# uber-research/vargp

Hardware: AMD Instinct MI355X
Metric: ELBO steps/sec (higher is better)
Workload: dtype f32; 1 GPU; BASELINE config 2 (Split-MNIST t=0): S3 F10 C10 M100 D784 B512 ELBO step; S_per_gpu=3, Mt=100, S_total=3, F=10, C=10, M=100, D=784, B=512, N=12000, optimizer=yogi, parallelism=sample-parallel x1, steps_per_graph_launch=10, launch=hipGraph replay

## Files before the change

vargp_amd/csrc/chol_blk16.h:

```cpp
#pragma once
#include "common.h"
#include <type_traits>

namespace vargp {

#ifdef VARGP_CB16_STAMPS
__device__ unsigned long long g_cb16_stamps[4][8][4];
extern "C" void vargp_debug_cb16_stamps(unsigned long long* out) { (void)hipMemcpyFromSymbol(out, HIP_SYMBOL(g_cb16_stamps), sizeof(g_cb16_stamps)); }
#define CB_STAMP(step, i) do { if (lane == 0 && blockIdx.x == 0) g_cb16_stamps[WV][step][i] = __builtin_amdgcn_s_memtime(); } while (0)
#else
#define CB_STAMP(step, i) do { } while (0)
#endif
typedef float cb_f32x4 __attribute__((ext_vector_type(4)));
constexpr int kCbNB = 7;
constexpr int kCbRD = 0;
constexpr int kCbWB = kCbRD + kCbNB * 256;
constexpr int kCbDD = kCbWB + 16 * 20;
constexpr int kCbED = kCbDD + 256;
constexpr int kCbLdsFloats = kCbED + 16;

template <int I, int N, class F>
__device__ __forceinline__ void cb_for(F&& f) {
  if constexpr (I < N) { f(std::integral_constant<int, I>{}); cb_for<I + 1, N>(f); }
}
__host__ __device__ constexpr int cb_owner(int c) { return c >= 3 ? 6 - c : c + 1; }
template <int WV> struct CbOwn {
  static constexpr int UA = 6 - WV, UB = WV > 0 ? WV - 1 : -1;
  static constexpr int XA = WV, XB = WV > 0 ? 7 - WV : -1;
  __host__ __device__ static constexpr bool owns_u(int c) { return c == UA || c == UB; }
  __host__ __device__ static constexpr bool owns_x(int c) { return c == XA || c == XB; }
  __host__ __device__ static constexpr int ui(int c, int k) { return c == UA ? k : (UA + 1) + k; }
  __host__ __device__ static constexpr int xi(int c, int i) { return c == XA ? i - XA : (7 - XA) + (i - XB); }
};

__device__ __forceinline__ void cb_mfma4(cb_f32x4& acc, const float4 a, const cb_f32x4 b) {
  acc = __builtin_amdgcn_mfma_f32_16x16x4f32(a.x, b[0], acc, 0, 0, 0);
  acc = __builtin_amdgcn_mfma_f32_16x16x4f32(a.y, b[1], acc, 0, 0, 0);
  acc = __builtin_amdgcn_mfma_f32_16x16x4f32(a.z, b[2], acc, 0, 0, 0);
  acc = __builtin_amdgcn_mfma_f32_16x16x4f32(a.w, b[3], acc, 0, 0, 0);
}
__device__ __forceinline__ void cb_barrier() { asm volatile("s_waitcnt lgkmcnt(0)\n\ts_barrier" ::: "memory"); }
__device__ __forceinline__ float cb_lane(float v, int lane) {
  return __int_as_float(__builtin_amdgcn_readlane(__float_as_int(v), lane));
}

template <int WV>
__device__ __forceinline__ void cb16_wave(float* __restrict__ stage, const int LS, double* __restrict__ sq, double* __restrict__ sd,
                                          const int n, const float eps, const int lane, int* __restrict__ flag, float* __restrict__ dump, int& fail) {
  using O = CbOwn<WV>;
  const int c = lane & 15, q = lane >> 4;
  cb_f32x4 accU[kCbNB], accX[kCbNB];
  cb_for<0, kCbNB>([&](auto ii) {
    constexpr int i = decltype(ii)::value;
    if constexpr (O::owns_u(i)) {
// ... 183 lines not shown
```

vargp_amd/csrc/common.h:

```cpp
#pragma once
#include <hip/hip_runtime.h>
#include <stdint.h>
#include <stdio.h>
#include <functional>
#include "../../include/vargp_hip.h"

#if defined(__HIPCC__)
namespace vargp {
constexpr int kSpanEnds = 4096;
struct SpanGuard {
  unsigned long long* p;
  unsigned long long* e;
  __device__ __forceinline__ SpanGuard(unsigned long long* q, unsigned long long* ends, int on) : p(on ? q : nullptr), e(ends) {
    if (p && threadIdx.x == 0 && blockIdx.x == 0 && blockIdx.y == 0 && blockIdx.z == 0) {
      p[0] = wall_clock64();
      p[2] = __builtin_amdgcn_s_memtime();
    }
  }
  __device__ __forceinline__ ~SpanGuard() {
    if (p && threadIdx.x == 0) {
      const unsigned lin = (blockIdx.z * gridDim.y + blockIdx.y) * gridDim.x + blockIdx.x;
      if (lin == 0) p[3] = __builtin_amdgcn_s_memtime();
      e[lin & (kSpanEnds - 1)] = wall_clock64();
    }
// ... 260 lines not shown
                     int D, int64_t Dp, int S, float kappa, int accumulate, hipStream_t st);

int chol_inv_bwd_first(const float* T, const float* gT, int nbatch, int n, void* ws, size_t ws_bytes,
                       const GemmParams* other, int oA, int oB, int onb, hipStream_t st);
int chol_inv_bwd_impl(const float* L, const float* T, const float* gL, const float* gT, float* gA, int nbatch, int n,
                      void* ws, size_t ws_bytes, bool gl_lower, hipStream_t st, bool first_done);

struct BwdMatArgs {
  const float* QP;
  const float *TT, *LL, *gQP, *RK, *KS, *seeds;
  const float* gTT;
  float *gKS, *Wuu, *r_uu, *gtheta;
  float *g_u_mean, *gLu_part;
  float* gL_acc;
  int S, C, M, D, NR, LD;
};
int launch_bwdmat_gemm(const BwdMatArgs& a, int first, int nmat, const GemmParams& p, int nbatch, hipStream_t st,
                       const char* tag, int* queue);

bool prof_remembering();
void prof_remember(const char* tag, std::function<void(hipStream_t)> relaunch);

struct ProfScope {
  ProfScope(const char* tag, hipStream_t st);
  ~ProfScope();
  int slot_;
  hipStream_t st_;
};

}
// ... 1 lines not shown
```

vargp_amd/csrc/elbo_t0.hip:

```cpp
#include <atomic>
#include <mutex>
#include <unordered_map>

#include "common.h"
STEP_SPAN_TABLE(t0)
#include "elbo_shared.h"
#include "t0_bwd_mid.h"
#include "t0_bwd_mid_multi.h"
#include "chol_gram.h"
#include "t0_prologue.h"
#include "t0_bwd_tail.h"

namespace vargp {

constexpr int kKuuSplit = 2;
#ifndef VARGP_KL_ROWS
#define VARGP_KL_ROWS 8
#endif
constexpr int kT0TileUnitsMax = 16384;
constexpr int kTailLdsDefault = 1;
constexpr int kKlRows = VARGP_KL_ROWS;


struct T0Ws {
// ... 850 lines not shown
                "%s: native noise needs rng_counter, eps_theta == eps_f == NULL and a sample offset >= 0", who);
  VARGP_REQUIRE(d->map_est ? d->S == 1
                           : (d->log_logvar && d->prior_log_mean && d->prior_log_logvar && (native || d->eps_theta)),
                "%s: hyper-parameter arguments inconsistent with map_est", who);
  VARGP_REQUIRE(d->ws_bytes >= vargp_elbo_t0_workspace_bytes(d->S, d->C, d->M, d->D, d->B, d->F),
                "%s: workspace too small", who);
  return VARGP_OK;
}

struct T0Tune {
  static long long env(const char* name, long long dflt) { const char* e = getenv(name); return e ? atoll(e) : dflt; }
  int64_t units = env("VARGP_T0_UNITS", kT0TileUnitsMax);
  int unmerge = env("VARGP_T0_UNMERGE", -1), side = env("VARGP_T0_SIDE", 1);
  int multi = env("VARGP_T0_MULTI", 0), parts = env("VARGP_T0_PARTS", 0);
  int fused = env("VARGP_T0_FUSED", 1), fused_bwd = env("VARGP_T0_FUSED_BWD", 1), mat_bwd = env("VARGP_T0_MAT_BWD", 1);
  int fold_small = env("VARGP_T0_FOLD_SMALL", 1);
  int front = env("VARGP_T0_FRONT", 1), gram_in_chain = env("VARGP_T0_GRAM_IN_CHAIN", -1), su = env("VARGP_T0_SU", 1);
  int tail = env("VARGP_T0_TAIL", 1), tail_lds = env("VARGP_T0_TAIL_LDS", kTailLdsDefault);
  int kuf_tile = env("VARGP_T0_KUF_TILE", 0), puf_tile = env("VARGP_T0_PUF_TILE", 0), puu_tile = env("VARGP_T0_PUU_TILE", 0);
  int kuu_split = env("VARGP_KUU_SPLIT", kKuuSplit), chol_f32 = env("VARGP_CHOL_F32", kCholF32Default);
};
static const T0Tune& t0_tune() { static const T0Tune tune; return tune; }

constexpr float kFwdMidSetup = 0.5f;
constexpr float kBwdMidSetup = 0.35f;
static int t0_tile_parts(int64_t SC, int ntile, int cus, float setup, int forced) {
  if (forced > 0) return forced < ntile ? forced : ntile;
  if (SC * ntile <= cus) return ntile;
  int best = ntile;
  float best_t = 1e30f;
  for (int np = 1; np <= ntile; ++np) {
    const float t = (float)cdiv(SC * np, (int64_t)cus) * (setup + (float)cdiv(ntile, np));
    if (t < best_t - 1e-6f) { best_t = t; best = np; }
  }
  return best;
}

struct T0Plan {
  bool native, generic_lik, unscaled_lik_grad, defer_softmax, fwd_softmax16;
  bool direct_gram, merge_chol, split_kuu, front, gram_in_chain, su_in_chain, fused_mid, fwd_multi, w_vec4;
  bool unmerge, side;
  bool fused_bwd, mat_bwd, bwd_multi, fused_tail, tail_lds;
  int kuf_tile, puf_tile, puu_tile;
  bool fold_small;
  int fold_roles, fold_extra;
  int ksp, ntile, fwd_parts, bwd_parts;
};
static T0Plan t0_plan(const vargp_elbo_t0_desc* d, const T0Ws& o, int cus) {
  const T0Tune& tune = t0_tune();
  const int S = d->S, C = d->C, M = d->M, D = d->D, B = d->B, F = d->F, LD = o.LD;
  const int64_t SC = (int64_t)S * C;
  const bool zx_aligned = ((reinterpret_cast<uintptr_t>(d->z) | reinterpret_cast<uintptr_t>(d->x)) & 15) == 0;
  T0Plan p{};
  p.native = t0_native(d);
  p.unscaled_lik_grad = C <= 16 && !d->ext_lik;
  p.generic_lik = C > 16 && !d->ext_lik;
  p.ntile = cdiv(B, 64);
// ... 15 lines not shown
  const bool units_ok = SC * p.ntile <= tune.units;
  p.fused_mid = tune.fused && M <= kFusedK && (M % 4) == 0 && (LD % 4) == 0 && units_ok;
  p.fwd_parts = t0_tile_parts(SC, p.ntile, cus, kFwdMidSetup, tune.parts);
  p.fwd_multi = p.fwd_parts < p.ntile || tune.multi == 1;
  p.w_vec4 = B % 4 == 0;
  {
    const int nsur = (int)(8 * cdiv(SC, 8) - SC) * p.ntile, need = (int)cdiv(SC, 2);
    p.fold_extra = nsur >= need ? 0 : (int)round_up(need - nsur, 8);
    p.fold_roles = nsur + p.fold_extra;
    p.fold_small = tune.fold_small && p.fused_mid && !p.fwd_multi && p.w_vec4 && !p.unmerge && M >= 4 &&
                   SC * p.ntile + std::min<int64_t>(p.fold_roles, SC) <= cus;
    if (!p.fold_small) p.fold_roles = p.fold_extra = 0;
  }
  p.fused_bwd = tune.fused_bwd && M <= kBmKP && M >= 4 && (M % 4) == 0 && (LD % 4) == 0 && (B % 4) == 0 && units_ok;
  p.mat_bwd = p.fused_bwd && tune.mat_bwd && (D % 4) == 0 && S <= kTailSMax && zx_aligned;
  p.bwd_parts = t0_tile_parts(SC, p.ntile, cus, kBwdMidSetup, tune.parts);
  p.bwd_multi = p.fused_bwd && (p.bwd_parts < p.ntile || tune.multi == 1);
  p.defer_softmax = d->defer_softmax && p.unscaled_lik_grad && p.fused_bwd && !p.bwd_multi && F <= 4 * kBmSmF && C <= kBmSmC &&
                    reinterpret_cast<uintptr_t>(p.native ? o.eps_f : d->eps_f) % 16 == 0;
  p.fwd_softmax16 = p.unscaled_lik_grad && !p.defer_softmax;
  p.fused_tail = p.mat_bwd && tune.tail && S <= kTailSMax;
  p.tail_lds = p.fused_tail && ((S > 4 && tune.tail_lds) || tune.tail_lds == 2);
  return p;
}

enum { kT0NoClear = 0, kT0Cleared = 1, kT0Consumed = 2, kT0SoftmaxDeferred = 16  };
static std::mutex g_t0_state_mu;
static std::unordered_map<const void*, int> g_t0_state;
static void t0_state_set(const void* ws, int v) {
  std::lock_guard<std::mutex> lock(g_t0_state_mu);
// ... 279 lines not shown
    ElboGemm gp{flat_gemm(o.QP + 4, LD, MLD, o.gW, B, MB, o.gQP + NR, LD, MLD, M, B, M), 0, 0, SC, "t0_gp_gemm"};
    gp.p.triA = 1;
    rc = run_gemm_pair(gg, gp.onto_c(), "t0_gg_gp_gemm", st);
    if (rc) return rc;
    rc = gt_gemm(false).run(st);
    if (rc) return rc;
    const ElboGemm grk = grk_gemm(NR + B);
    rc = chol_inv_bwd_first(o.TT, o.gTT, SC + C, M, o.chol, o.chol_bytes, &grk.p, grk.tA, grk.tB, grk.nbatch, st);
    if (rc) return rc;
  }
  if (plan.mat_bwd) {
    BwdMatArgs ma{};
    ma.QP = o.QP; ma.TT = o.TT; ma.LL = o.LL; ma.gQP = o.gQP; ma.RK = o.RK; ma.KS = o.KS; ma.seeds = seeds; ma.gTT = o.gTT;
    ma.gKS = o.gKS; ma.Wuu = o.Wuu; ma.r_uu = o.r_uu; ma.gtheta = o.gtheta;
    ma.g_u_mean = g_u_mean; ma.gLu_part = o.gLL;
    ma.S = S; ma.C = C; ma.M = M; ma.D = D; ma.NR = NR; ma.LD = LD;
    GemmParams puf = puf_gemm();
    if (plan.unmerge) {
      SideFork fork(st, plan.side);
      ma.gL_acc = o.gLL + SC * MM;
      rc = launch_bwdmat_gemm(ma, 0, SC, puf, 0, fork.side(), "t0_bwdmat_kuu", nullptr);
      if (rc) return rc;
      rc = launch_bwdmat_gemm(ma, SC, C, puf, 0, fork.side(), "t0_bwdmat_su", nullptr);
      if (rc) return rc;
      puf.tile = plan.puf_tile;
      rc = launch_gemm(puf, 0, 0, S, false, st, "rbf_kuf_bwd_product");
      if (rc) return rc;
      rc = fork.join();
    } else {
      rc = launch_bwdmat_gemm(ma, 0, SC + C, puf, S, st, "rbf_kuf_bwd_gemm", reinterpret_cast<int*>(o.queue));
    }
// ... 108 lines not shown
```

vargp_amd/csrc/gemm.hip:

```cpp
#include "common.h"
#include "chol_small3.h"
#include "t0_bwd_mat.h"
#include "t0_prologue.h"
#include <atomic>
#include <stdlib.h>
#include <string.h>
#include <type_traits>

STEP_SPAN_TABLE(gemm)
#ifdef STEP_SPANS
__device__ unsigned long long g_bmat_ends[64][2];
extern "C" void vargp_debug_bmat_ends(unsigned long long* out) { (void)hipMemcpyFromSymbol(out, HIP_SYMBOL(g_bmat_ends), sizeof(g_bmat_ends)); }
#endif

namespace vargp {

typedef float f32x16 __attribute__((ext_vector_type(16)));

__device__ float g_gemm_trash[512];

template <bool KC, int ROWS, int BK>
struct LdsLayout {
  static constexpr int kStride = KC ? BK : (ROWS + 4);
  static constexpr int kSize = KC ? ROWS * BK : BK * (ROWS + 4);
// ... 1294 lines not shown
  return check_launch("gemm_pair2");
}

static bool gemm_persist_ok(const GemmParams& p, int BK, bool AKC, bool BKC) {
  const int64_t extA = AKC ? ((int64_t)(p.M - 1) * p.lda + p.K) : ((int64_t)(p.K - 1) * p.lda + p.M);
  const int64_t extB = BKC ? ((int64_t)(p.N - 1) * p.ldb + p.K) : ((int64_t)(p.K - 1) * p.ldb + p.N);
  return gemm_vec_ok(p) && p.K >= 4 * BK && p.K % BK == 0 && !p.D && p.triA == 0 && p.triB == 0 && p.triC == 0 && !p.symout &&
         p.splitk <= 1 && (AKC || (p.M % 4 == 0 && p.M >= 4)) && (BKC || (p.N % 4 == 0 && p.N >= 4)) &&
         extA < (1ll << 29) && extB < (1ll << 29);
}

int launch_bwdmat_gemm(const BwdMatArgs& a, int first, int nmat, const GemmParams& p, int nbatch, hipStream_t st,
                       const char* tag, int* queue) {
  VARGP_REQUIRE(gemm_vec_ok(p), "bwdmat_gemm: the product's operands must be 16-byte aligned with strides % 4 == 0");
  VARGP_REQUIRE(a.M <= kBmKP && a.M >= 4 && (a.M % 4) == 0 && (a.LD % 4) == 0, "bwdmat_gemm: M = %d out of range", a.M);
  static_assert(kBwdMatLdsBytes >= sizeof(float) * gemm_lds_floats<64, 64, 64, true, false>(), "LDS of the GEMM role");
  if (prof_remembering() && strcmp(tag, "replay") != 0) {
    const GemmParams pc = p;
    const BwdMatArgs ac = a;
    prof_remember(tag, [=](hipStream_t s) { launch_bwdmat_gemm(ac, first, nmat, pc, nbatch, s, "replay", nullptr); });
  }
  static std::atomic<unsigned> attr_mask[2] = {};
  int dev = 0;
  VARGP_REQUIRE(hipGetDevice(&dev) == hipSuccess && dev >= 0 && dev < 64, "bwdmat_gemm: hipGetDevice failed");
  if (!((attr_mask[dev >> 5].load(std::memory_order_acquire) >> (dev & 31)) & 1u)) {
    VARGP_REQUIRE(hipFuncSetAttribute(reinterpret_cast<const void*>(t0_bwdmat_gemm_kernel),
                                      hipFuncAttributeMaxDynamicSharedMemorySize, (int)kBwdMatLdsBytes) == hipSuccess,
                  "bwdmat_gemm: cannot reserve %zu bytes of LDS", kBwdMatLdsBytes);
    attr_mask[dev >> 5].fetch_or(1u << (dev & 31), std::memory_order_release);
  }
// ... 88 lines not shown
```

vargp_amd/csrc/t0_bwd_mat.h:

```cpp
#pragma once
#include "t0_bwd_common.h"

namespace vargp {

constexpr int kMatS = 108;
constexpr int kMatN = kBmKP * kMatS;
constexpr size_t kBwdMatLdsBytes = sizeof(float) * (3 * kMatN + 4 * 128 + 8);

enum { kFamL = 0, kFamR = 1, kFamC = 2, kFamF = 3 };
constexpr unsigned kNone = 0xFFu;
__host__ __device__ constexpr unsigned mat_blk(int rb, int cb) { return (unsigned)((rb << 2) | cb); }
__host__ __device__ constexpr unsigned mat_blk4(unsigned a, unsigned b, unsigned c, unsigned d) {
  return a | (b << 8) | (c << 16) | (d << 24);
}
__host__ __device__ constexpr unsigned mat_blocks(int family, int wave) {
  return family == kFamL
             ? (wave == 0   ? mat_blk4(mat_blk(3, 3), mat_blk(0, 0), mat_blk(1, 0), kNone)
                : wave == 1 ? mat_blk4(mat_blk(2, 2), mat_blk(1, 1), kNone, kNone)
                : wave == 2 ? mat_blk4(mat_blk(3, 2), mat_blk(2, 1), kNone, kNone)
                            : mat_blk4(mat_blk(3, 1), mat_blk(2, 0), mat_blk(3, 0), kNone))
         : family == kFamR
             ? (wave == 0   ? mat_blk4(mat_blk(0, 0), mat_blk(3, 0), mat_blk(3, 1), kNone)
                : wave == 1 ? mat_blk4(mat_blk(1, 0), mat_blk(2, 0), kNone, kNone)
                : wave == 2 ? mat_blk4(mat_blk(1, 1), mat_blk(2, 1), kNone, kNone)
                            : mat_blk4(mat_blk(2, 2), mat_blk(3, 2), mat_blk(3, 3), kNone))
         : family == kFamC
             ? (wave == 0   ? mat_blk4(mat_blk(0, 0), mat_blk(1, 1), kNone, kNone)
                : wave == 1 ? mat_blk4(mat_blk(1, 0), mat_blk(2, 1), kNone, kNone)
                : wave == 2 ? mat_blk4(mat_blk(2, 0), mat_blk(3, 1), kNone, kNone)
                            : mat_blk4(mat_blk(3, 0), mat_blk(2, 2), mat_blk(3, 2), mat_blk(3, 3)))
             : (wave == 0   ? mat_blk4(mat_blk(0, 0), mat_blk(0, 1), mat_blk(3, 0), mat_blk(3, 1))
                : wave == 1 ? mat_blk4(mat_blk(0, 2), mat_blk(0, 3), mat_blk(3, 2), mat_blk(3, 3))
                : wave == 2 ? mat_blk4(mat_blk(1, 0), mat_blk(1, 1), mat_blk(2, 0), mat_blk(2, 1))
                            : mat_blk4(mat_blk(1, 2), mat_blk(1, 3), mat_blk(2, 2), mat_blk(2, 3)));
}
template <int FAM, int WV, int U> struct MatBlk {
  static constexpr unsigned code = (mat_blocks(FAM, WV) >> (8 * U)) & 0xFFu;
  static constexpr bool valid = code != kNone;
  static constexpr int rb = valid ? (int)(code >> 2) : 0, cb = valid ? (int)(code & 3u) : 0;
  static constexpr int GE = kBmKP / 8;
  static constexpr int g0 = FAM == kFamL ? 0 : (FAM == kFamC ? 4 * cb : 4 * rb);
  static constexpr int g1 = FAM == kFamL ? bm_min(GE, 4 * cb + 4) : GE;
};

template <bool AKC, bool BKC, int RB, int CB, int G0, int G1>
__device__ __forceinline__ void mat_block(bm_f32x16& acc, const float* __restrict__ sA, const float* __restrict__ sB, int li, int lh) {
  const int ia = min(32 * RB + li, kBmKP - 1), ib = min(32 * CB + li, kBmKP - 1);
  const float* pa = AKC ? sA + ia * kMatS + 4 * lh : sA + (4 * lh) * kMatS + ia;
  const float* pb = BKC ? sB + ib * kMatS + 4 * lh : sB + (4 * lh) * kMatS + ib;
  auto fa = [&](int g) { return AKC ? bm_frag_kc(pa, 8 * g) : bm_frag_km(pa, 8 * g, kMatS); };
  auto fb = [&](int g) { return BKC ? bm_frag_kc(pb, 8 * g) : bm_frag_km(pb, 8 * g, kMatS); };
  float4 a = fa(G0), b = fb(G0);
  bm_for<G0, G1>([&](auto gi) {
    constexpr int g = decltype(gi)::value;
    const float4 ca = a, cbv = b;
    if constexpr (g + 1 < G1) { a = fa(g + 1); b = fb(g + 1); }
    bm_mfma4(acc, ca, cbv);
  });
}

template <bool AKC, bool BKC, int FAM, int WV>
__device__ __forceinline__ void mat_product(bm_f32x16 (&acc)[4], const float* __restrict__ sA, const float* __restrict__ sB,
                                            bool zero, int li, int lh) {
  bm_for<0, 4>([&](auto ui) {
    constexpr int u = decltype(ui)::value;
    using Bk = MatBlk<FAM, WV, u>;
    if constexpr (Bk::valid) {
      if (zero) {
#pragma unroll
        for (int r = 0; r < 16; ++r) acc[u][r] = 0.f;
      }
      mat_block<AKC, BKC, Bk::rb, Bk::cb, Bk::g0, Bk::g1>(acc[u], sA, sB, li, lh);
    }
  });
}
template <int FAM, int WV, class F>
__device__ __forceinline__ void mat_foreach(int li, int lh, F&& f) {
  bm_for<0, 4>([&](auto ui) {
    constexpr int u = decltype(ui)::value;
    using Bk = MatBlk<FAM, WV, u>;
    if constexpr (Bk::valid) {
#pragma unroll
      for (int r = 0; r < 16; ++r) f(u, Bk::rb, Bk::cb, r, 32 * Bk::rb + (r & 3) + 8 * (r >> 2) + 4 * lh, 32 * Bk::cb + li);
    }
  });
}

__device__ __forceinline__ void mat_store(float* __restrict__ dst, const float4 (&src)[kBmNA], int M, int tid) {
#pragma unroll
  for (int u = 0; u < kBmNA; ++u) {
    const int e = tid + 256 * u;
    const int i = e / kBmNQ, j = (e - i * kBmNQ) * 4;
    const float4 v = (i < M && j < M) ? src[u] : make_float4(0.f, 0.f, 0.f, 0.f);
    if (e < kBmKP * kBmNQ) *reinterpret_cast<float4*>(&dst[i * kMatS + j]) = v;
  }
}

#ifdef BMAT_STAMPS
// ... 3 lines not shown
  if (reset) {
    const unsigned long long init[2][4] = {{~0ull, 0, 0, 0}, {~0ull, 0, 0, 0}};
    (void)hipMemcpyToSymbol(HIP_SYMBOL(g_bmat_span), init, sizeof(init));
  } else {
    (void)hipMemcpyFromSymbol(out, HIP_SYMBOL(g_bmat_span), 64);
  }
}
extern "C" void vargp_debug_bmat_stamps(unsigned long long* out) { (void)hipMemcpyFromSymbol(out, HIP_SYMBOL(g_bmat_stamps), 4 * 192); }
#define BMAT_STAMP(i) do { if ((threadIdx.x & 63) == 0 && id == 0) g_bmat_stamps[threadIdx.x >> 6][i] = __builtin_amdgcn_s_memtime(); } while (0)
#define BSU_STAMP(i) do { if (threadIdx.x == 0 && id == a.S * a.C) g_bmat_stamps[3][17 + (i)] = __builtin_amdgcn_s_memtime(); } while (0)
#else
#define BMAT_STAMP(i) do { } while (0)
#define BSU_STAMP(i) do { } while (0)
#endif

template <int FAM, int WV>
__device__ __forceinline__ void mat_write_sym(float* __restrict__ X, const bm_f32x16 (&acc)[4], int M, float scale, float diag,
                                              int li, int lh) {
  bm_for<0, 4>([&](auto ui) {
    constexpr int u = decltype(ui)::value;
    using Bk = MatBlk<FAM, WV, u>;
    if constexpr (Bk::valid) {
      const int j = 32 * Bk::cb + li;
      if constexpr (Bk::rb != Bk::cb) {
#pragma unroll
        for (int q = 0; q < 4; ++q) {
          const int i0 = 32 * Bk::rb + 8 * q + 4 * lh;
          float v[4];
#pragma unroll
          for (int t = 0; t < 4; ++t) v[t] = i0 + t < M ? scale * acc[u][4 * q + t] : 0.f;
          if (i0 < kBmKP) {
#pragma unroll
            for (int t = 0; t < 4; ++t) X[(i0 + t) * kMatS + j] = v[t];
            *reinterpret_cast<float4*>(&X[j * kMatS + i0]) = make_float4(v[0], v[1], v[2], v[3]);
          }
        }
      } else {
#pragma unroll
        for (int r = 0; r < 16; ++r) {
          const int i = 32 * Bk::rb + (r & 3) + 8 * (r >> 2) + 4 * lh;
          if (i < kBmKP && j <= i) {
            const float v = i < M ? scale * ((i == j ? diag : 0.f) + acc[u][r]) : 0.f;
            X[i * kMatS + j] = v;
            X[j * kMatS + i] = v;
          }
        }
      }
    }
  });
}

template <int WV>
__device__ __forceinline__ void mat_tail(float* __restrict__ sT, float* __restrict__ X1, float* __restrict__ X2,
                                         const float* __restrict__ kmul, float* __restrict__ out, float* __restrict__ rsum_out,
                                         float* __restrict__ tot_out, int M, int id, int tid, int lane, int li, int lh) {
  bm_f32x16 acc[4];
  float4 kr[kBmNA];
  if (kmul) bm_load_mat(kmul, M, M, tid, kr);
  mat_product<false, true, kFamF, WV>(acc, sT, X2, true, li, lh);
  BMAT_STAMP(12);
  __syncthreads();
  mat_foreach<kFamF, WV>(li, lh, [&](int u, int rb, int cb, int r, int i, int j) {
    if (i < kBmKP && j < kBmKP) X1[i * kMatS + j] = i < M ? acc[u][r] : 0.f;
  });
  __syncthreads();
  BMAT_STAMP(13);
  mat_product<true, false, kFamC, WV>(acc, X1, sT, true, li, lh);
  BMAT_STAMP(14);
  mat_write_sym<kFamC, WV>(X2, acc, M, 1.f, 0.f, li, lh);
  __syncthreads();
  BMAT_STAMP(15);
  float dsum = 0.f;
  float4 xv[kBmNA];
#pragma unroll
  for (int u = 0; u < kBmNA; ++u) {
    const int e = min(tid + 256 * u, kBmKP * kBmNQ - 1);
    const int i = e / kBmNQ, j = (e - i * kBmNQ) * 4;
    xv[u] = *reinterpret_cast<const float4*>(&X2[i * kMatS + j]);
  }
#pragma unroll
  for (int u = 0; u < kBmNA; ++u) {
    const int e = tid + 256 * u;
    const int i = e / kBmNQ, j = (e - i * kBmNQ) * 4;
    float4 v = xv[u];
// ... 16 lines not shown
#pragma unroll
    for (int q = 0; q < 13; ++q) {
      const float4 v = *reinterpret_cast<const float4*>(pr + 4 * q);
      a0 += v.x + v.z; a1 += v.y + v.w;
    }
    float t = a0 + a1;
    t += __shfl_xor(t, 1, 64);
    if (h == 0 && i < M) rsum_out[(int64_t)id * M + i] = t;
    float tot = ((h == 0 && i < M) ? t : 0.f) + dsum;
    tot = wave_sum(tot);
    if (lane == 0) atomicAdd(tot_out, tot);
  }
  BMAT_STAMP(16);
}

template <int WV>
__device__ __forceinline__ void mat_kuu(const BwdMatArgs& a, int id, float* __restrict__ lds, int tid, int lane, int li, int lh) {
  float* sT = lds;
  float* X1 = sT + kMatN;
  float* X2 = X1 + kMatN;
  float* sga = X2 + kMatN;
  float* smv = sga + 128;
  float* srs = smv + 128;
  const int M = a.M, LD = a.LD;
  const int64_t MM = (int64_t)M * M, MLD = (int64_t)M * LD;
  const int64_t b = id;
  const int c = id % a.C;
  const float* Tb = a.TT + b * MM;
  const float* gq = a.gQP + b * MLD;
  const float* qp = a.QP + b * MLD;
  const float* rk = a.RK + b * MLD;
  const float g = a.seeds[1] / (float)a.S;
  bm_f32x16 acc[4];
  float4 r0[kBmNA], r1[kBmNA], r2[kBmNA];
  BMAT_STAMP(0);
  bm_load_mat(gq + 4, LD, M, tid, r1);
  bm_load_mat(rk + 4, LD, M, tid, r2);
  bm_load_mat(Tb, M, M, tid, r0);
  const float gav = tid < 128 ? gq[(int64_t)min(tid, M - 1) * LD] + g * qp[(int64_t)min(tid, M - 1) * LD] : 0.f;
  const float mvv = tid < 128 ? rk[(int64_t)min(tid, M - 1) * LD] : 0.f;
  mat_store(X1, r1, M, tid);
  mat_store(X2, r2, M, tid);
  bm_load_mat(qp + 4 + M, LD, M, tid, r1);
  bm_load_mat(rk + 4 + M, LD, M, tid, r2);
  float gtt[4][16];
  {
    const float* gTb = a.gTT + b * MM;
    mat_foreach<kFamL, WV>(li, lh, [&](int u, int rb, int cb, int r, int i, int j) {
      gtt[u][r] = gTb[(int64_t)min(i, M - 1) * M + min(j, M - 1)];
    });
  }
  __syncthreads();
  BMAT_STAMP(1);
  mat_product<true, true, kFamL, WV>(acc, X1, X2, true, li, lh);
  BMAT_STAMP(2);
  mat_store(sT, r0, M, tid);
  if (tid < 128) { sga[tid] = tid < M ? gav : 0.f; smv[tid] = tid < M ? mvv : 0.f; }
  __syncthreads();
  BMAT_STAMP(3);
  if (a.gL_acc) {
    bm_f32x16 acx[4];
    mat_product<false, false, kFamR, WV>(acx, sT, X1, true, li, lh);
    float* gl = a.gL_acc + (int64_t)c * MM;
    mat_foreach<kFamR, WV>(li, lh, [&](int u, int rb, int cb, int r, int i, int j) {
      if (i < M && (rb != cb || j <= i)) atomicAdd(&gl[(int64_t)i * M + j], acx[u][r]);
    });
    __syncthreads();
  }
#pragma unroll
  for (int u = 0; u < kBmNA; ++u) { r1[u].x *= g; r1[u].y *= g; r1[u].z *= g; r1[u].w *= g; }
  mat_store(X1, r1, M, tid);
  mat_store(X2, r2, M, tid);
  {
    const int i = tid & 127, h = tid >> 7, ic = min(i, kBmKP - 1);
    constexpr int KH = kBmKP / 2;
    const float* tp = sT + (KH * h) * kMatS + ic;
    float tv[KH];
    float4 gk[KH / 4];
#pragma unroll
// ... 3 lines not shown
    float s0 = 0.f, s1 = 0.f;
#pragma unroll
    for (int q = 0; q < KH / 4; ++q) {
      const int k0 = KH * h + 4 * q;
      s0 = fmaf(k0 >= i ? tv[4 * q] : 0.f, gk[q].x, s0);
      s1 = fmaf(k0 + 1 >= i ? tv[4 * q + 1] : 0.f, gk[q].y, s1);
      s0 = fmaf(k0 + 2 >= i ? tv[4 * q + 2] : 0.f, gk[q].z, s0);
      s1 = fmaf(k0 + 3 >= i ? tv[4 * q + 3] : 0.f, gk[q].w, s1);
    }
    srs[tid] = s0 + s1;
  }
  __syncthreads();
  BMAT_STAMP(5);
  if (tid < M) atomicAdd(&a.g_u_mean[(int64_t)c * M + tid], srs[tid] + srs[tid + 128]);
  BMAT_STAMP(6);
  mat_product<true, true, kFamL, WV>(acc, X1, X2, false, li, lh);
  {
    bm_f32x16 acr[4];
    mat_product<false, false, kFamR, WV>(acr, sT, X1, true, li, lh);
    float* gl = a.gLu_part + b * MM;
    mat_foreach<kFamR, WV>(li, lh, [&](int u, int rb, int cb, int r, int i, int j) {
      if (i < M && (rb != cb || j <= i)) gl[(int64_t)i * M + j] = acr[u][r];
    });
  }
  BMAT_STAMP(7);
  __syncthreads();
  BMAT_STAMP(8);
  float gai[4][16], mj[4];
  mat_foreach<kFamL, WV>(li, lh, [&](int u, int rb, int cb, int r, int i, int j) {
    gai[u][r] = sga[i];
    if (r == 0) mj[u] = smv[j];
  });
  mat_foreach<kFamL, WV>(li, lh, [&](int u, int rb, int cb, int r, int i, int j) {
    const float v = acc[u][r] + gtt[u][r] + gai[u][r] * mj[u];
    if (i < kBmKP && j < kBmKP) X1[i * kMatS + j] = (i < M && j <= i) ? v : 0.f;
  });
  __syncthreads();
  BMAT_STAMP(9);
  mat_product<true, true, kFamL, WV>(acc, X1, sT, true, li, lh);
  BMAT_STAMP(10);
  mat_write_sym<kFamL, WV>(X2, acc, M, -0.5f, -g, li, lh);
  __syncthreads();
  BMAT_STAMP(11);
  mat_tail<WV>(sT, X1, X2, a.KS + b * MM, a.Wuu + b * MM, a.r_uu, &a.gtheta[(int64_t)(id / a.C) * (a.D + 1) + a.D], M, id, tid,
               lane, li, lh);
}

template <int WV>
__device__ __forceinline__ void mat_su(const BwdMatArgs& a, int id, float* __restrict__ lds, int tid, int lane, int li, int lh) {
  float* sT = lds;
  float* X1 = sT + kMatN;
  float* X2 = X1 + kMatN;
  const int M = a.M, LD = a.LD, SC = a.S * a.C;
  const int64_t MM = (int64_t)M * M, MLD = (int64_t)M * LD;
  const int c = id - SC;
  bm_f32x16 acc[4];
  float4 r0[kBmNA], r1[kBmNA];
  BSU_STAMP(0);
  if (a.gL_acc) {
    bm_load_mat(a.TT + (int64_t)id * MM, M, M, tid, r0);
    bm_load_mat(a.LL + (int64_t)id * MM, M, M, tid, r1);
    const float* gl = a.gL_acc + (int64_t)c * MM;
    mat_foreach<kFamR, WV>(li, lh, [&](int u, int rb, int cb, int r, int i, int j) {
      acc[u][r] = gl[(int64_t)min(i, M - 1) * M + min(j, M - 1)];
    });
  } else {
  bm_load_mat(a.TT + (int64_t)c * MM, M, M, tid, r0);
  bm_load_mat(a.gQP + (int64_t)c * MLD + 4, LD, M, tid, r1);
  }
  for (int s = 0; s < (a.gL_acc ? 0 : a.S); ++s) {
    if (s > 0) __syncthreads();
    mat_store(sT, r0, M, tid);
    mat_store(X1, r1, M, tid);
    __syncthreads();
    const bool more = s + 1 < a.S;
    const int64_t bn = (int64_t)(s + 1) * a.C + c;
    bm_load_mat(a.TT + (more ? bn : (int64_t)id) * MM, M, M, tid, r0);
    bm_load_mat(more ? a.gQP + bn * MLD + 4 : a.LL + (int64_t)id * MM, more ? LD : M, M, tid, r1);
    mat_product<false, false, kFamR, WV>(acc, sT, X1, s == 0, li, lh);
  }
  BSU_STAMP(1);
  __syncthreads();
  mat_foreach<kFamR, WV>(li, lh, [&](int u, int rb, int cb, int r, int i, int j) {
    if (i < kBmKP && j < kBmKP) X2[i * kMatS + j] = (i < M && j <= i) ? acc[u][r] : 0.f;
  });
  mat_store(sT, r0, M, tid);
  mat_store(X1, r1, M, tid);
  __syncthreads();
  BSU_STAMP(2);
  mat_product<false, false, kFamR, WV>(acc, X1, X2, true, li, lh);
  __syncthreads();
  mat_write_sym<kFamR, WV>(X2, acc, M, 0.5f, 0.f, li, lh);
  __syncthreads();
  BSU_STAMP(3);
  mat_tail<WV>(sT, X1, X2, nullptr, a.gKS + (int64_t)id * MM, nullptr, nullptr, M, id, tid, lane, li, lh);
  BSU_STAMP(4);
}

__device__ __forceinline__ void t0_bwd_mat_body(const BwdMatArgs& a, int id, float* __restrict__ lds) {
  const int tid = threadIdx.x, lane = tid & 63, wave = tid >> 6, li = lane & 31, lh = lane >> 5;
  if (id < a.S * a.C) {
    if (wave == 0) mat_kuu<0>(a, id, lds, tid, lane, li, lh);
    else if (wave == 1) mat_kuu<1>(a, id, lds, tid, lane, li, lh);
    else if (wave == 2) mat_kuu<2>(a, id, lds, tid, lane, li, lh);
    else mat_kuu<3>(a, id, lds, tid, lane, li, lh);
  } else {
    if (wave == 0) mat_su<0>(a, id, lds, tid, lane, li, lh);
    else if (wave == 1) mat_su<1>(a, id, lds, tid, lane, li, lh);
    else if (wave == 2) mat_su<2>(a, id, lds, tid, lane, li, lh);
    else mat_su<3>(a, id, lds, tid, lane, li, lh);
  }
}

}
```

Measured before the change: 5663 ELBO steps/s (Cfg2 step: S=3 hyper-samples).

## Add 16x16 MFMA tiling with balanced block tables to fused backward matrix kernel

Adds a 16x16x4 MFMA cut for the per-sample matrix products in the fused backward kernel. Work is assigned by a compile-time greedy load-balanced table of 16-blocks per wave, with a three-deep register prefetch of LDS fragments and a half-width last K group to cover the 104-wide padding. It becomes the default, with the old 32-block path kept behind an environment switch. The aim is to cut wasted MFMA work on triangular and padded blocks and to balance load across the four waves. The cost is more accumulator registers, more instructions, and scattered LDS fragment reads.

```diff
diff --git a/vargp_amd/csrc/chol_blk16.h b/vargp_amd/csrc/chol_blk16.h
--- a/vargp_amd/csrc/chol_blk16.h
+++ b/vargp_amd/csrc/chol_blk16.h
@@ -38,6 +38,10 @@
   acc = __builtin_amdgcn_mfma_f32_16x16x4f32(a.y, b[1], acc, 0, 0, 0);
   acc = __builtin_amdgcn_mfma_f32_16x16x4f32(a.z, b[2], acc, 0, 0, 0);
   acc = __builtin_amdgcn_mfma_f32_16x16x4f32(a.w, b[3], acc, 0, 0, 0);
+}
+__device__ __forceinline__ void cb_mfma2(cb_f32x4& acc, const float a0, const float a1, const float b0, const float b1) {
+  acc = __builtin_amdgcn_mfma_f32_16x16x4f32(a0, b0, acc, 0, 0, 0);
+  acc = __builtin_amdgcn_mfma_f32_16x16x4f32(a1, b1, acc, 0, 0, 0);
 }
 __device__ __forceinline__ void cb_barrier() { asm volatile("s_waitcnt lgkmcnt(0)\n\ts_barrier" ::: "memory"); }
 __device__ __forceinline__ float cb_lane(float v, int lane) {
diff --git a/vargp_amd/csrc/common.h b/vargp_amd/csrc/common.h
--- a/vargp_amd/csrc/common.h
+++ b/vargp_amd/csrc/common.h
@@ -298,6 +298,7 @@
   float *g_u_mean, *gLu_part;
   float* gL_acc;
   int S, C, M, D, NR, LD;
+  int blk;
 };
 int launch_bwdmat_gemm(const BwdMatArgs& a, int first, int nmat, const GemmParams& p, int nbatch, hipStream_t st,
                        const char* tag, int* queue);
diff --git a/vargp_amd/csrc/elbo_t0.hip b/vargp_amd/csrc/elbo_t0.hip
--- a/vargp_amd/csrc/elbo_t0.hip
+++ b/vargp_amd/csrc/elbo_t0.hip
@@ -888,6 +888,7 @@
   int unmerge = env("VARGP_T0_UNMERGE", -1), side = env("VARGP_T0_SIDE", 1);
   int multi = env("VARGP_T0_MULTI", 0), parts = env("VARGP_T0_PARTS", 0);
   int fused = env("VARGP_T0_FUSED", 1), fused_bwd = env("VARGP_T0_FUSED_BWD", 1), mat_bwd = env("VARGP_T0_MAT_BWD", 1);
+  int mat_blk = env("VARGP_T0_MAT_BLK", 16);
   int fold_small = env("VARGP_T0_FOLD_SMALL", 1);
   int front = env("VARGP_T0_FRONT", 1), gram_in_chain = env("VARGP_T0_GRAM_IN_CHAIN", -1), su = env("VARGP_T0_SU", 1);
   int tail = env("VARGP_T0_TAIL", 1), tail_lds = env("VARGP_T0_TAIL_LDS", kTailLdsDefault);
@@ -915,6 +916,7 @@
   bool direct_gram, merge_chol, split_kuu, front, gram_in_chain, su_in_chain, fused_mid, fwd_multi, w_vec4;
   bool unmerge, side;
   bool fused_bwd, mat_bwd, bwd_multi, fused_tail, tail_lds;
+  int mat_blk;
   int kuf_tile, puf_tile, puu_tile;
   bool fold_small;
   int fold_roles, fold_extra;
@@ -960,6 +962,7 @@
   }
   p.fused_bwd = tune.fused_bwd && M <= kBmKP && M >= 4 && (M % 4) == 0 && (LD % 4) == 0 && (B % 4) == 0 && units_ok;
   p.mat_bwd = p.fused_bwd && tune.mat_bwd && (D % 4) == 0 && S <= kTailSMax && zx_aligned;
+  p.mat_blk = tune.mat_blk == 32 ? 32 : 16;
   p.bwd_parts = t0_tile_parts(SC, p.ntile, cus, kBwdMidSetup, tune.parts);
   p.bwd_multi = p.fused_bwd && (p.bwd_parts < p.ntile || tune.multi == 1);
   p.defer_softmax = d->defer_softmax && p.unscaled_lik_grad && p.fused_bwd && !p.bwd_multi && F <= 4 * kBmSmF && C <= kBmSmC &&
@@ -1269,7 +1272,7 @@
     ma.QP = o.QP; ma.TT = o.TT; ma.LL = o.LL; ma.gQP = o.gQP; ma.RK = o.RK; ma.KS = o.KS; ma.seeds = seeds; ma.gTT = o.gTT;
     ma.gKS = o.gKS; ma.Wuu = o.Wuu; ma.r_uu = o.r_uu; ma.gtheta = o.gtheta;
     ma.g_u_mean = g_u_mean; ma.gLu_part = o.gLL;
-    ma.S = S; ma.C = C; ma.M = M; ma.D = D; ma.NR = NR; ma.LD = LD;
+    ma.S = S; ma.C = C; ma.M = M; ma.D = D; ma.NR = NR; ma.LD = LD; ma.blk = plan.mat_blk;
     GemmParams puf = puf_gemm();
     if (plan.unmerge) {
       SideFork fork(st, plan.side);
diff --git a/vargp_amd/csrc/gemm.hip b/vargp_amd/csrc/gemm.hip
--- a/vargp_amd/csrc/gemm.hip
+++ b/vargp_amd/csrc/gemm.hip
@@ -1332,6 +1332,7 @@
                        const char* tag, int* queue) {
   VARGP_REQUIRE(gemm_vec_ok(p), "bwdmat_gemm: the product's operands must be 16-byte aligned with strides % 4 == 0");
   VARGP_REQUIRE(a.M <= kBmKP && a.M >= 4 && (a.M % 4) == 0 && (a.LD % 4) == 0, "bwdmat_gemm: M = %d out of range", a.M);
+  VARGP_REQUIRE(a.blk == 16 || a.blk == 32, "bwdmat_gemm: block size %d is neither 16 nor 32", a.blk);
   static_assert(kBwdMatLdsBytes >= sizeof(float) * gemm_lds_floats<64, 64, 64, true, false>(), "LDS of the GEMM role");
   if (prof_remembering() && strcmp(tag, "replay") != 0) {
     const GemmParams pc = p;
diff --git a/vargp_amd/csrc/t0_bwd_mat.h b/vargp_amd/csrc/t0_bwd_mat.h
--- a/vargp_amd/csrc/t0_bwd_mat.h
+++ b/vargp_amd/csrc/t0_bwd_mat.h
@@ -1,5 +1,6 @@
 #pragma once
 #include "t0_bwd_common.h"
+#include "chol_blk16.h"
 
 namespace vargp {
 
@@ -34,13 +35,63 @@
                 : wave == 2 ? mat_blk4(mat_blk(1, 0), mat_blk(1, 1), mat_blk(2, 0), mat_blk(2, 1))
                             : mat_blk4(mat_blk(1, 2), mat_blk(1, 3), mat_blk(2, 2), mat_blk(2, 3)));
 }
-template <int FAM, int WV, int U> struct MatBlk {
-  static constexpr unsigned code = (mat_blocks(FAM, WV) >> (8 * U)) & 0xFFu;
+template <int BLK> struct MatCut;
+template <> struct MatCut<32> { using Acc = bm_f32x16; static constexpr int NU = 4, NR = 16; };
+template <> struct MatCut<16> { using Acc = cb_f32x4; static constexpr int NU = 14, NR = 4; };
+template <int BLK>
+__device__ __forceinline__ int mat_row(int rb, int r, int lh) {
+  return BLK == 32 ? 32 * rb + (r & 3) + 8 * (r >> 2) + 4 * lh : 16 * rb + 4 * lh + r;
+}
+
+template <int BLK, int FAM, int WV, int U> struct MatBlk;
+template <int FAM, int WV, int U> struct MatBlk<32, FAM, WV, U> {
+  static constexpr unsigned code = U < 4 ? (mat_blocks(FAM, WV) >> (8 * (U & 3))) & 0xFFu : kNone;
   static constexpr bool valid = code != kNone;
   static constexpr int rb = valid ? (int)(code >> 2) : 0, cb = valid ? (int)(code & 3u) : 0;
   static constexpr int GE = kBmKP / 8;
   static constexpr int g0 = FAM == kFamL ? 0 : (FAM == kFamC ? 4 * cb : 4 * rb);
   static constexpr int g1 = FAM == kFamL ? bm_min(GE, 4 * cb + 4) : GE;
+};
+
+constexpr int kMat16NB = 7, kMat16NG = 7;
+static_assert(kBmKP == 16 * (kMat16NG - 1) + 8, "the 16 cut's last K group is a half group");
+__host__ __device__ constexpr int mat16_g0(int fam, int rb, int cb) { return fam == kFamL ? 0 : (fam == kFamC ? cb : rb); }
+__host__ __device__ constexpr int mat16_g1(int fam, int rb, int cb) { return fam == kFamL ? cb + 1 : kMat16NG; }
+__host__ __device__ constexpr int mat16_cost(int fam, int rb, int cb) {
+  return 2 * (mat16_g1(fam, rb, cb) - mat16_g0(fam, rb, cb)) - (mat16_g1(fam, rb, cb) == kMat16NG ? 1 : 0);
+}
+struct MatTab16 { unsigned char blk[4][MatCut<16>::NU]; int n[4]; int load[4]; };
+__host__ __device__ constexpr MatTab16 mat16_table(int fam) {
+  MatTab16 t{};
+  for (int cost = 2 * kMat16NG; cost >= 1; --cost)
+    for (int rb = 0; rb < kMat16NB; ++rb)
+      for (int cb = 0; cb <= (fam == kFamF ? kMat16NB - 1 : rb); ++cb) {
+        if (mat16_cost(fam, rb, cb) != cost) continue;
+        int w = 0;
+        for (int v = 1; v < 4; ++v)
+          if (t.load[v] < t.load[w] || (t.load[v] == t.load[w] && t.n[v] < t.n[w])) w = v;
+        t.blk[w][t.n[w]++] = (unsigned char)((rb << 3) | cb);
+        t.load[w] += cost;
+      }
+  return t;
+}
+struct MatSteps16 { unsigned char u[112], g[112]; int n; };
+__host__ __device__ constexpr MatSteps16 mat16_steps(int fam, int wave) {
+  const MatTab16 t = mat16_table(fam);
+  MatSteps16 s{};
+  for (int u = 0; u < t.n[wave]; ++u) {
+    const int rb = t.blk[wave][u] >> 3, cb = t.blk[wave][u] & 7;
+    for (int g = mat16_g0(fam, rb, cb); g < mat16_g1(fam, rb, cb); ++g) { s.u[s.n] = (unsigned char)u; s.g[s.n] = (unsigned char)g; ++s.n; }
+  }
+  return s;
+}
+template <int FAM, int WV> struct MatWave16 {
+  static constexpr MatTab16 tab = mat16_table(FAM);
+  static constexpr MatSteps16 st = mat16_steps(FAM, WV);
+};
+template <int FAM, int WV, int U> struct MatBlk<16, FAM, WV, U> {
+  static constexpr bool valid = U < MatWave16<FAM, WV>::tab.n[WV];
+  static constexpr int rb = valid ? MatWave16<FAM, WV>::tab.blk[WV][U] >> 3 : 0, cb = valid ? MatWave16<FAM, WV>::tab.blk[WV][U] & 7 : 0;
 };
 
 template <bool AKC, bool BKC, int RB, int CB, int G0, int G1>
@@ -59,29 +110,83 @@
   });
 }
 
+template <bool KC, int IB, int G>
+__device__ __forceinline__ float4 mat16_frag(const float* __restrict__ s, int li, int lh) {
+  const int idx = IB == kMat16NB - 1 ? min(16 * IB + li, kBmKP - 1) : 16 * IB + li;
+  if constexpr (G < kMat16NG - 1) {
+    if constexpr (KC) {
+      return *reinterpret_cast<const float4*>(s + idx * kMatS + 16 * G + 4 * lh);
+    } else {
+      const float* p = s + (16 * G + 4 * lh) * kMatS + idx;
+      return make_float4(p[0], p[kMatS], p[2 * kMatS], p[3 * kMatS]);
+    }
+  } else {
+    if constexpr (KC) {
+      const float2 v = *reinterpret_cast<const float2*>(s + idx * kMatS + 16 * G + 2 * lh);
+      return make_float4(v.x, v.y, 0.f, 0.f);
+    } else {
+      const float* p = s + (16 * G + 2 * lh) * kMatS + idx;
+      return make_float4(p[0], p[kMatS], 0.f, 0.f);
+    }
+  }
+}
 template <bool AKC, bool BKC, int FAM, int WV>
-__device__ __forceinline__ void mat_product(bm_f32x16 (&acc)[4], const float* __restrict__ sA, const float* __restrict__ sB,
-                                            bool zero, int li, int lh) {
-  bm_for<0, 4>([&](auto ui) {
+__device__ __forceinline__ void mat_product16(cb_f32x4 (&acc)[MatCut<16>::NU], const float* __restrict__ sA,
+                                              const float* __restrict__ sB, bool zero, int li, int lh) {
+  using W = MatWave16<FAM, WV>;
+  constexpr int NS = W::st.n;
+  static_assert(NS > 2, "every wave has blocks in every family");
+  if (zero) {
+    bm_for<0, MatCut<16>::NU>([&](auto ui) {
+      constexpr int u = decltype(ui)::value;
+      if constexpr (MatBlk<16, FAM, WV, u>::valid) acc[u] = cb_f32x4{0.f, 0.f, 0.f, 0.f};
+    });
+  }
+  float4 fa[3], fb[3];
+  auto request = [&](auto si) {
+    constexpr int s = decltype(si)::value, u = W::st.u[s], g = W::st.g[s];
+    using Bk = MatBlk<16, FAM, WV, u>;
+    fa[s % 3] = mat16_frag<AKC, Bk::rb, g>(sA, li, lh);
+    fb[s % 3] = mat16_frag<BKC, Bk::cb, g>(sB, li, lh);
+  };
+  request(std::integral_constant<int, 0>{});
+  request(std::integral_constant<int, 1>{});
+  bm_for<0, NS>([&](auto si) {
+    constexpr int s = decltype(si)::value, u = W::st.u[s], g = W::st.g[s];
+    const float4 a = fa[s % 3], b = fb[s % 3];
+    if constexpr (s + 2 < NS) request(std::integral_constant<int, s + 2>{});
+    if constexpr (g < kMat16NG - 1) cb_mfma4(acc[u], a, cb_f32x4{b.x, b.y, b.z, b.w});
+    else cb_mfma2(acc[u], a.x, a.y, b.x, b.y);
+  });
+}
+
+template <int BLK, bool AKC, bool BKC, int FAM, int WV>
+__device__ __forceinline__ void mat_product(typename MatCut<BLK>::Acc (&acc)[MatCut<BLK>::NU], const float* __restrict__ sA,
+                                            const float* __restrict__ sB, bool zero, int li, int lh) {
+  if constexpr (BLK == 16) {
+    mat_product16<AKC, BKC, FAM, WV>(acc, sA, sB, zero, li, lh);
+  } else {
+    bm_for<0, 4>([&](auto ui) {
+      constexpr int u = decltype(ui)::value;
+      using Bk = MatBlk<32, FAM, WV, u>;
+      if constexpr (Bk::valid) {
+        if (zero) {
+#pragma unroll
+          for (int r = 0; r < 16; ++r) acc[u][r] = 0.f;
+        }
+        mat_block<AKC, BKC, Bk::rb, Bk::cb, Bk::g0, Bk::g1>(acc[u], sA, sB, li, lh);
+      }
+    });
+  }
+}
+template <int BLK, int FAM, int WV, class F>
+__device__ __forceinline__ void mat_foreach(int li, int lh, F&& f) {
+  bm_for<0, MatCut<BLK>::NU>([&](auto ui) {
     constexpr int u = decltype(ui)::value;
-    using Bk = MatBlk<FAM, WV, u>;
+    using Bk = MatBlk<BLK, FAM, WV, u>;
     if constexpr (Bk::valid) {
-      if (zero) {
-#pragma unroll
-        for (int r = 0; r < 16; ++r) acc[u][r] = 0.f;
-      }
-      mat_block<AKC, BKC, Bk::rb, Bk::cb, Bk::g0, Bk::g1>(acc[u], sA, sB, li, lh);
-    }
-  });
-}
-template <int FAM, int WV, class F>
-__device__ __forceinline__ void mat_foreach(int li, int lh, F&& f) {
-  bm_for<0, 4>([&](auto ui) {
-    constexpr int u = decltype(ui)::value;
-    using Bk = MatBlk<FAM, WV, u>;
-    if constexpr (Bk::valid) {
-#pragma unroll
-      for (int r = 0; r < 16; ++r) f(u, Bk::rb, Bk::cb, r, 32 * Bk::rb + (r & 3) + 8 * (r >> 2) + 4 * lh, 32 * Bk::cb + li);
+#pragma unroll
+      for (int r = 0; r < MatCut<BLK>::NR; ++r) f(u, Bk::rb, Bk::cb, r, mat_row<BLK>(Bk::rb, r, lh), BLK * Bk::cb + li);
     }
   });
 }
@@ -115,18 +220,18 @@
 #define BSU_STAMP(i) do { } while (0)
 #endif
 
-template <int FAM, int WV>
-__device__ __forceinline__ void mat_write_sym(float* __restrict__ X, const bm_f32x16 (&acc)[4], int M, float scale, float diag,
-                                              int li, int lh) {
-  bm_for<0, 4>([&](auto ui) {
+template <int BLK, int FAM, int WV>
+__device__ __forceinline__ void mat_write_sym(float* __restrict__ X, const typename MatCut<BLK>::Acc (&acc)[MatCut<BLK>::NU], int M,
+                                              float scale, float diag, int li, int lh) {
+  bm_for<0, MatCut<BLK>::NU>([&](auto ui) {
     constexpr int u = decltype(ui)::value;
-    using Bk = MatBlk<FAM, WV, u>;
+    using Bk = MatBlk<BLK, FAM, WV, u>;
     if constexpr (Bk::valid) {
-      const int j = 32 * Bk::cb + li;
+      const int j = BLK * Bk::cb + li;
       if constexpr (Bk::rb != Bk::cb) {
 #pragma unroll
-        for (int q = 0; q < 4; ++q) {
-          const int i0 = 32 * Bk::rb + 8 * q + 4 * lh;
+        for (int q = 0; q < MatCut<BLK>::NR / 4; ++q) {
+          const int i0 = mat_row<BLK>(Bk::rb, 4 * q, lh);
           float v[4];
 #pragma unroll
           for (int t = 0; t < 4; ++t) v[t] = i0 + t < M ? scale * acc[u][4 * q + t] : 0.f;
@@ -138,8 +243,8 @@
         }
       } else {
 #pragma unroll
-        for (int r = 0; r < 16; ++r) {
-          const int i = 32 * Bk::rb + (r & 3) + 8 * (r >> 2) + 4 * lh;
+        for (int r = 0; r < MatCut<BLK>::NR; ++r) {
+          const int i = mat_row<BLK>(Bk::rb, r, lh);
           if (i < kBmKP && j <= i) {
             const float v = i < M ? scale * ((i == j ? diag : 0.f) + acc[u][r]) : 0.f;
             X[i * kMatS + j] = v;
@@ -151,24 +256,24 @@
   });
 }
 
-template <int WV>
+template <int BLK, int WV>
 __device__ __forceinline__ void mat_tail(float* __restrict__ sT, float* __restrict__ X1, float* __restrict__ X2,
                                          const float* __restrict__ kmul, float* __restrict__ out, float* __restrict__ rsum_out,
                                          float* __restrict__ tot_out, int M, int id, int tid, int lane, int li, int lh) {
-  bm_f32x16 acc[4];
+  typename MatCut<BLK>::Acc acc[MatCut<BLK>::NU];
   float4 kr[kBmNA];
   if (kmul) bm_load_mat(kmul, M, M, tid, kr);
-  mat_product<false, true, kFamF, WV>(acc, sT, X2, true, li, lh);
+  mat_product<BLK, false, true, kFamF, WV>(acc, sT, X2, true, li, lh);
   BMAT_STAMP(12);
   __syncthreads();
-  mat_foreach<kFamF, WV>(li, lh, [&](int u, int rb, int cb, int r, int i, int j) {
+  mat_foreach<BLK, kFamF, WV>(li, lh, [&](int u, int rb, int cb, int r, int i, int j) {
     if (i < kBmKP && j < kBmKP) X1[i * kMatS + j] = i < M ? acc[u][r] : 0.f;
   });
   __syncthreads();
   BMAT_STAMP(13);
-  mat_product<true, false, kFamC, WV>(acc, X1, sT, true, li, lh);
+  mat_product<BLK, true, false, kFamC, WV>(acc, X1, sT, true, li, lh);
   BMAT_STAMP(14);
-  mat_write_sym<kFamC, WV>(X2, acc, M, 1.f, 0.f, li, lh);
+  mat_write_sym<BLK, kFamC, WV>(X2, acc, M, 1.f, 0.f, li, lh);
   __syncthreads();
   BMAT_STAMP(15);
   float dsum = 0.f;
@@ -215,7 +320,7 @@
   BMAT_STAMP(16);
 }
 
-template <int WV>
+template <int BLK, int WV>
 __device__ __forceinline__ void mat_kuu(const BwdMatArgs& a, int id, float* __restrict__ lds, int tid, int lane, int li, int lh) {
   float* sT = lds;
   float* X1 = sT + kMatN;
@@ -232,7 +337,7 @@
   const float* qp = a.QP + b * MLD;
   const float* rk = a.RK + b * MLD;
   const float g = a.seeds[1] / (float)a.S;
-  bm_f32x16 acc[4];
+  typename MatCut<BLK>::Acc acc[MatCut<BLK>::NU];
   float4 r0[kBmNA], r1[kBmNA], r2[kBmNA];
   BMAT_STAMP(0);
   bm_load_mat(gq + 4, LD, M, tid, r1);
@@ -244,26 +349,26 @@
   mat_store(X2, r2, M, tid);
   bm_load_mat(qp + 4 + M, LD, M, tid, r1);
   bm_load_mat(rk + 4 + M, LD, M, tid, r2);
-  float gtt[4][16];
+  float gtt[MatCut<BLK>::NU][MatCut<BLK>::NR];
   {
     const float* gTb = a.gTT + b * MM;
-    mat_foreach<kFamL, WV>(li, lh, [&](int u, int rb, int cb, int r, int i, int j) {
+    mat_foreach<BLK, kFamL, WV>(li, lh, [&](int u, int rb, int cb, int r, int i, int j) {
       gtt[u][r] = gTb[(int64_t)min(i, M - 1) * M + min(j, M - 1)];
     });
   }
   __syncthreads();
   BMAT_STAMP(1);
-  mat_product<true, true, kFamL, WV>(acc, X1, X2, true, li, lh);
+  mat_product<BLK, true, true, kFamL, WV>(acc, X1, X2, true, li, lh);
   BMAT_STAMP(2);
   mat_store(sT, r0, M, tid);
   if (tid < 128) { sga[tid] = tid < M ? gav : 0.f; smv[tid] = tid < M ? mvv : 0.f; }
   __syncthreads();
   BMAT_STAMP(3);
   if (a.gL_acc) {
-    bm_f32x16 acx[4];
-    mat_product<false, false, kFamR, WV>(acx, sT, X1, true, li, lh);
+    typename MatCut<BLK>::Acc acx[MatCut<BLK>::NU];
+    mat_product<BLK, false, false, kFamR, WV>(acx, sT, X1, true, li, lh);
     float* gl = a.gL_acc + (int64_t)c * MM;
-    mat_foreach<kFamR, WV>(li, lh, [&](int u, int rb, int cb, int r, int i, int j) {
+    mat_foreach<BLK, kFamR, WV>(li, lh, [&](int u, int rb, int cb, int r, int i, int j) {
       if (i < M && (rb != cb || j <= i)) atomicAdd(&gl[(int64_t)i * M + j], acx[u][r]);
     });
     __syncthreads();
@@ -297,39 +402,39 @@
   BMAT_STAMP(5);
   if (tid < M) atomicAdd(&a.g_u_mean[(int64_t)c * M + tid], srs[tid] + srs[tid + 128]);
   BMAT_STAMP(6);
-  mat_product<true, true, kFamL, WV>(acc, X1, X2, false, li, lh);
+  mat_product<BLK, true, true, kFamL, WV>(acc, X1, X2, false, li, lh);
   {
-    bm_f32x16 acr[4];
-    mat_product<false, false, kFamR, WV>(acr, sT, X1, true, li, lh);
+    typename MatCut<BLK>::Acc acr[MatCut<BLK>::NU];
+    mat_product<BLK, false, false, kFamR, WV>(acr, sT, X1, true, li, lh);
     float* gl = a.gLu_part + b * MM;
-    mat_foreach<kFamR, WV>(li, lh, [&](int u, int rb, int cb, int r, int i, int j) {
+    mat_foreach<BLK, kFamR, WV>(li, lh, [&](int u, int rb, int cb, int r, int i, int j) {
       if (i < M && (rb != cb || j <= i)) gl[(int64_t)i * M + j] = acr[u][r];
     });
   }
   BMAT_STAMP(7);
   __syncthreads();
   BMAT_STAMP(8);
-  float gai[4][16], mj[4];
-  mat_foreach<kFamL, WV>(li, lh, [&](int u, int rb, int cb, int r, int i, int j) {
+  float gai[MatCut<BLK>::NU][MatCut<BLK>::NR], mj[MatCut<BLK>::NU];
+  mat_foreach<BLK, kFamL, WV>(li, lh, [&](int u, int rb, int cb, int r, int i, int j) {
     gai[u][r] = sga[i];
     if (r == 0) mj[u] = smv[j];
   });
-  mat_foreach<kFamL, WV>(li, lh, [&](int u, int rb, int cb, int r, int i, int j) {
+  mat_foreach<BLK, kFamL, WV>(li, lh, [&](int u, int rb, int cb, int r, int i, int j) {
     const float v = acc[u][r] + gtt[u][r] + gai[u][r] * mj[u];
     if (i < kBmKP && j < kBmKP) X1[i * kMatS + j] = (i < M && j <= i) ? v : 0.f;
   });
   __syncthreads();
   BMAT_STAMP(9);
-  mat_product<true, true, kFamL, WV>(acc, X1, sT, true, li, lh);
+  mat_product<BLK, true, true, kFamL, WV>(acc, X1, sT, true, li, lh);
   BMAT_STAMP(10);
-  mat_write_sym<kFamL, WV>(X2, acc, M, -0.5f, -g, li, lh);
+  mat_write_sym<BLK, kFamL, WV>(X2, acc, M, -0.5f, -g, li, lh);
   __syncthreads();
   BMAT_STAMP(11);
-  mat_tail<WV>(sT, X1, X2, a.KS + b * MM, a.Wuu + b * MM, a.r_uu, &a.gtheta[(int64_t)(id / a.C) * (a.D + 1) + a.D], M, id, tid,
+  mat_tail<BLK, WV>(sT, X1, X2, a.KS + b * MM, a.Wuu + b * MM, a.r_uu, &a.gtheta[(int64_t)(id / a.C) * (a.D + 1) + a.D], M, id, tid,
                lane, li, lh);
 }
 
-template <int WV>
+template <int BLK, int WV>
 __device__ __forceinline__ void mat_su(const BwdMatArgs& a, int id, float* __restrict__ lds, int tid, int lane, int li, int lh) {
   float* sT = lds;
   float* X1 = sT + kMatN;
@@ -337,14 +442,14 @@
   const int M = a.M, LD = a.LD, SC = a.S * a.C;
   const int64_t MM = (int64_t)M * M, MLD = (int64_t)M * LD;
   const int c = id - SC;
-  bm_f32x16 acc[4];
+  typename MatCut<BLK>::Acc acc[MatCut<BLK>::NU];
   float4 r0[kBmNA], r1[kBmNA];
   BSU_STAMP(0);
   if (a.gL_acc) {
     bm_load_mat(a.TT + (int64_t)id * MM, M, M, tid, r0);
     bm_load_mat(a.LL + (int64_t)id * MM, M, M, tid, r1);
     const float* gl = a.gL_acc + (int64_t)c * MM;
-    mat_foreach<kFamR, WV>(li, lh, [&](int u, int rb, int cb, int r, int i, int j) {
+    mat_foreach<BLK, kFamR, WV>(li, lh, [&](int u, int rb, int cb, int r, int i, int j) {
       acc[u][r] = gl[(int64_t)min(i, M - 1) * M + min(j, M - 1)];
     });
   } else {
@@ -360,39 +465,44 @@
     const int64_t bn = (int64_t)(s + 1) * a.C + c;
     bm_load_mat(a.TT + (more ? bn : (int64_t)id) * MM, M, M, tid, r0);
     bm_load_mat(more ? a.gQP + bn * MLD + 4 : a.LL + (int64_t)id * MM, more ? LD : M, M, tid, r1);
-    mat_product<false, false, kFamR, WV>(acc, sT, X1, s == 0, li, lh);
+    mat_product<BLK, false, false, kFamR, WV>(acc, sT, X1, s == 0, li, lh);
   }
   BSU_STAMP(1);
   __syncthreads();
-  mat_foreach<kFamR, WV>(li, lh, [&](int u, int rb, int cb, int r, int i, int j) {
+  mat_foreach<BLK, kFamR, WV>(li, lh, [&](int u, int rb, int cb, int r, int i, int j) {
     if (i < kBmKP && j < kBmKP) X2[i * kMatS + j] = (i < M && j <= i) ? acc[u][r] : 0.f;
   });
   mat_store(sT, r0, M, tid);
   mat_store(X1, r1, M, tid);
   __syncthreads();
   BSU_STAMP(2);
-  mat_product<false, false, kFamR, WV>(acc, X1, X2, true, li, lh);
-  __syncthreads();
-  mat_write_sym<kFamR, WV>(X2, acc, M, 0.5f, 0.f, li, lh);
+  mat_product<BLK, false, false, kFamR, WV>(acc, X1, X2, true, li, lh);
+  __syncthreads();
+  mat_write_sym<BLK, kFamR, WV>(X2, acc, M, 0.5f, 0.f, li, lh);
   __syncthreads();
   BSU_STAMP(3);
-  mat_tail<WV>(sT, X1, X2, nullptr, a.gKS + (int64_t)id * MM, nullptr, nullptr, M, id, tid, lane, li, lh);
+  mat_tail<BLK, WV>(sT, X1, X2, nullptr, a.gKS + (int64_t)id * MM, nullptr, nullptr, M, id, tid, lane, li, lh);
   BSU_STAMP(4);
 }
 
+template <int BLK>
+__device__ __forceinline__ void t0_bwd_mat_cut(const BwdMatArgs& a, int id, float* __restrict__ lds) {
+  const int tid = threadIdx.x, lane = tid & 63, wave = tid >> 6, li = lane & (BLK - 1), lh = lane / BLK;
+  if (id < a.S * a.C) {
+    if (wave == 0) mat_kuu<BLK, 0>(a, id, lds, tid, lane, li, lh);
+    else if (wave == 1) mat_kuu<BLK, 1>(a, id, lds, tid, lane, li, lh);
+    else if (wave == 2) mat_kuu<BLK, 2>(a, id, lds, tid, lane, li, lh);
+    else mat_kuu<BLK, 3>(a, id, lds, tid, lane, li, lh);
+  } else {
+    if (wave == 0) mat_su<BLK, 0>(a, id, lds, tid, lane, li, lh);
+    else if (wave == 1) mat_su<BLK, 1>(a, id, lds, tid, lane, li, lh);
+    else if (wave == 2) mat_su<BLK, 2>(a, id, lds, tid, lane, li, lh);
+    else mat_su<BLK, 3>(a, id, lds, tid, lane, li, lh);
+  }
+}
 __device__ __forceinline__ void t0_bwd_mat_body(const BwdMatArgs& a, int id, float* __restrict__ lds) {
-  const int tid = threadIdx.x, lane = tid & 63, wave = tid >> 6, li = lane & 31, lh = lane >> 5;
-  if (id < a.S * a.C) {
-    if (wave == 0) mat_kuu<0>(a, id, lds, tid, lane, li, lh);
-    else if (wave == 1) mat_kuu<1>(a, id, lds, tid, lane, li, lh);
-    else if (wave == 2) mat_kuu<2>(a, id, lds, tid, lane, li, lh);
-    else mat_kuu<3>(a, id, lds, tid, lane, li, lh);
-  } else {
-    if (wave == 0) mat_su<0>(a, id, lds, tid, lane, li, lh);
-    else if (wave == 1) mat_su<1>(a, id, lds, tid, lane, li, lh);
-    else if (wave == 2) mat_su<2>(a, id, lds, tid, lane, li, lh);
-    else mat_su<3>(a, id, lds, tid, lane, li, lh);
-  }
-}
-
-}
+  if (a.blk == 32) t0_bwd_mat_cut<32>(a, id, lds);
+  else t0_bwd_mat_cut<16>(a, id, lds);
+}
+
+}
```

Result: no change. 5683 ELBO steps/s (Cfg2 step: S=3 hyper-samples), median of 6 (+0.4%).
